# ngrabaskas/Torch-Automatic-Distributed-Neural-Network

Measured on AMD Instinct MI355X. Metric: samples/sec whole-node ResNet-50 DP + GPT-2 PP at 1/2/4/8 MI355X; scaling eff, higher is better.
Workload: dtype bf16

## Files before the change

madnn/ops/__init__.py:

```python
from __future__ import annotations

import os
import threading
from pathlib import Path
from typing import Optional, Sequence

import torch
import torch.nn.functional as F

from . import reference

HERE = Path(__file__).resolve().parent
_KERNELS = HERE / "_madnn_kernels.so"
_lock = threading.Lock()
_loaded = {"kernels": False, "error": None}


def kernels_path() -> Path:
    return _KERNELS


class StaleKernelsError(RuntimeError):
    """The in-tree kernel library was built from different sources than the tree holds."""

# ... 545 lines not shown
    return torch.cat([a * c - b * sn, b * c + a * sn], -1).to(x.dtype)


class _RopeQKVFn(torch.autograd.Function):

    @staticmethod
    def forward(ctx, qkv, cos, sin, rot_heads):
        ctx.save_for_backward(cos, sin)
        ctx.rot = rot_heads
        if _is_dev(qkv):
            return torch.ops.madnn.rope_qkv(qkv, cos, sin, rot_heads, False)
        out = qkv.clone()
        out[:, :, :rot_heads] = _rope_rotate(qkv[:, :, :rot_heads], cos, sin, False)
        return out

    @staticmethod
    def backward(ctx, g):
        cos, sin = ctx.saved_tensors
        g = g.contiguous()
        if _is_dev(g):
            torch.ops.madnn.rope_qkv_(g, cos, sin, ctx.rot, True)
        else:
            g = g.clone()
            g[:, :, : ctx.rot] = _rope_rotate(g[:, :, : ctx.rot], cos, sin, True)
        return g, None, None, None


def rope_qkv(qkv: torch.Tensor, cos: torch.Tensor, sin: torch.Tensor, rot_heads: int) -> torch.Tensor:
    if _is_dev(qkv):
        _need_native("rope_qkv")
        if not (qkv.dtype == torch.bfloat16 and qkv.is_contiguous() and qkv.size(-1) % 16 == 0
                and cos.dtype == torch.float32 and cos.is_contiguous()):
            raise ValueError("rope_qkv: needs a contiguous bf16 qkv (D % 16 == 0) and fp32 tables")
        if qkv.data_ptr() % 16:
            qkv = qkv.clone()
        if cos.data_ptr() % 16 or sin.data_ptr() % 16:
            cos, sin = cos.clone(), sin.clone()
    return _RopeQKVFn.apply(qkv, cos, sin, rot_heads)


class _SwiGLUFn(torch.autograd.Function):

    @staticmethod
    def forward(ctx, gu):
        ctx.save_for_backward(gu)
        return torch.ops.madnn.swiglu_fwd(gu)

    @staticmethod
    def backward(ctx, dh):
        (gu,) = ctx.saved_tensors
        if dh.data_ptr() % 16 or not dh.is_contiguous():
            dh = dh.contiguous().clone()
        return torch.ops.madnn.swiglu_bwd(dh, gu)


def swiglu(gu: torch.Tensor) -> torch.Tensor:
    if (_is_dev(gu) and gu.dtype == torch.bfloat16 and gu.is_contiguous() and gu.size(-1) % 16 == 0
            and gu.data_ptr() % 16 == 0):
        _need_native("swiglu")
        return _SwiGLUFn.apply(gu)
    g, u = gu.chunk(2, dim=-1)
    return F.silu(g) * u


def _nhwc(t: torch.Tensor) -> torch.Tensor:
    return t.contiguous(memory_format=torch.channels_last) if t.dim() == 4 else t.contiguous()


def _rows(t: torch.Tensor) -> torch.Tensor:
    return t.permute(0, 2, 3, 1).reshape(-1, t.size(1)) if t.dim() == 4 else t


def conv1x1_route(cin: int, cout: int) -> tuple:
    fwd = "k9" if (cin <= 256 or cout >= 2 * cin) else "miopen"
    if _K9_DGRAD == "narrow":
        dgrad = "k9" if (cin <= 256 and cout <= 512) else "gemm"
    else:
        dgrad = "gemm" if (cout >= 1024 and cout >= 4 * cin) else "k9"
    return fwd, dgrad, _K9_WGRAD


_K9_WGRAD = os.environ.get("MADNN_K9_WGRAD", "miopen")
_K9_DGRAD = os.environ.get("MADNN_K9_DGRAD", "narrow")


def _routed_conv1x1_fwd(fwd: str, x: torch.Tensor, w: torch.Tensor, stats: bool):
    if fwd == "k9":
        return torch.ops.madnn.conv1x1_fwd(x, w, bool(stats))
    y = F.conv2d(x, w) if x.dim() == 4 else torch.mm(x, w.reshape(w.size(0), -1).t())
    return y, x.new_empty((0, 2, w.size(0)), dtype=torch.float32)


def _routed_conv1x1_wgrad(wgrad: str, dy: torch.Tensor, x: torch.Tensor, w: torch.Tensor) -> torch.Tensor:
    return _k9_wgrad(dy, x, w) if wgrad == "k9" else _conv1x1_wgrad_lib(dy, x, w)


def _with_stats(out: torch.Tensor, part: torch.Tensor, stats: bool):
    return (out, part if part.numel() else None) if stats else out


def _like(g: torch.Tensor, y: torch.Tensor) -> torch.Tensor:
    return g if g.dtype == y.dtype and g.stride() == y.stride() else torch.empty_like(y).copy_(g)


class _Conv1x1Fn(torch.autograd.Function):

    @staticmethod
    def forward(ctx, x, w, stats, fork):
        fwd, dgrad, wgrad = conv1x1_route(x.size(1), w.size(0))
        y, part = _routed_conv1x1_fwd(fwd, x, w, stats)
        ctx.save_for_backward(x, w)
        ctx.route = (dgrad, wgrad)
        ctx.fork = fork
        ctx.mark_non_differentiable(part)
        if fork == 2:
            return y, part, x[:, :, ::2, ::2].contiguous(memory_format=torch.channels_last)
        if fork:
            return y, part, x.view_as(x)
        return y, part

    @staticmethod
    def backward(ctx, dy, _dpart, dfork=None):
        x, w = ctx.saved_tensors
        dgrad, wgrad = ctx.route
        dy = _nhwc(dy.to(x.dtype))
        sub = None
        if ctx.fork == 2:
            sub, dfork = dfork, None
        resmask = _attached(dfork, "_madnn_resmask", strict=True)
        res = _nhwc(dfork.to(x.dtype)) if dfork is not None else None
        if resmask is not None and not (ctx.needs_input_grad[0] and dgrad == "k9"):
            res, resmask = _apply_bit_mask(res, resmask), None
        dx = dw = None
        if ctx.needs_input_grad[0]:
            if dgrad == "k9":
                dx = torch.ops.madnn.conv1x1_dgrad(dy, w, res, resmask)
            else:
                w2 = w.reshape(w.size(0), -1)
                if res is not None:
                    dx = res if res._base is None else _nhwc(res.clone())
                    _rows(dx).addmm_(_rows(dy), w2)
                else:
                    dx = torch.empty_like(x)
                    torch.mm(_rows(dy), w2, out=_rows(dx))
        elif res is not None:
            dx = res
        if sub is not None:
            if dx is None:
                dx = torch.zeros_like(x)
            dx[:, :, ::2, ::2].add_(sub.to(dx.dtype))
        if ctx.needs_input_grad[1]:
            dw = _routed_conv1x1_wgrad(wgrad, dy, x, w)
        return dx, dw, None, None


def conv1x1_supported(x: torch.Tensor, w: torch.Tensor) -> bool:
    if x.device.type != "cuda" or x.dtype != torch.bfloat16 or w.dtype != torch.bfloat16 or x.numel() == 0:
        return False
    if x.dim() == 4:
        if not x.is_contiguous(memory_format=torch.channels_last):
            return False
    elif x.dim() != 2 or not x.is_contiguous():
        return False
    cin, cout = x.size(1), w.size(0)
    if w.numel() != cin * cout or w.stride(0) != cin or w.stride(1) != 1:
        return False
    return cin % 64 == 0 and cout % 64 == 0


def conv1x1(x: torch.Tensor, w: torch.Tensor, *, stats: bool = False, fork: bool = False):
    _need_native("conv1x1")
    y, part, *side = _Conv1x1Fn.apply(x, w, stats, fork)
    ret = (y, part if part.numel() else None, *side) if stats else (y, *side)
    return ret[0] if len(ret) == 1 else ret


class _BNReluConv1x1EpiFn(torch.autograd.Function):

    @staticmethod
    def forward(ctx, y, w, bn_w, bn_b, bn, stats_in, want_stats):
        a, mean, invstd, scale, shift, _ = _bn_fwd_train(y, None, bn_w, bn_b, bn, True, stats_in)
        fwd, _, wgrad = conv1x1_route(a.size(1), w.size(0))
        out, part = _routed_conv1x1_fwd(fwd, a, w, want_stats)
        ctx.save_for_backward(y, a, w, bn_w, mean, invstd, scale, shift)
        ctx.wgrad = wgrad
        ctx.mark_non_differentiable(part)
        return out, part

    @staticmethod
    def backward(ctx, dout, _dpart):
        y, a, w, bn_w, mean, invstd, scale, shift = ctx.saved_tensors
        dout = _nhwc(dout.to(y.dtype))
        da, part = torch.ops.madnn.conv1x1_dgrad_bnb(dout, w, y, scale, shift)
        dw = _routed_conv1x1_wgrad(ctx.wgrad, dout, a, w)
        dy, dbw, dbb = torch.ops.madnn.bn_bwd_ext(da, y, bn_w, mean, invstd, scale, shift, part, True)
        need_bn = ctx.needs_input_grad[2] or ctx.needs_input_grad[3]
        return dy, dw, dbw if need_bn else None, dbb if need_bn else None, None, None, None


def bn_relu_conv1x1(y: torch.Tensor, bn, w: torch.Tensor, *, stats_in: Optional[torch.Tensor] = None,
                    stats: bool = False, checked: bool = False):
    if checked or bn_relu_conv1x1_epi_supported(y, bn, w):
        _need_native("bn_relu_conv1x1")
        return _with_stats(*_BNReluConv1x1EpiFn.apply(y, w, bn.weight, bn.bias, bn, stats_in, stats), stats)
    a = bn(y, relu=True, stats=stats_in) if _is_fused_bn(bn) else torch.relu(bn(y))
    if conv1x1_supported(a, w):
        return conv1x1(a, w, stats=stats)
    out = torch.nn.functional.conv2d(a, w.view(w.size(0), -1, 1, 1)) if a.dim() == 4 else torch.mm(
        a, w.reshape(w.size(0), -1).t())
    return (out, None) if stats else out


def bn_relu_conv1x1_epi_supported(y: torch.Tensor, bn, w: torch.Tensor) -> bool:
    return (_BN_DGRAD_EPI and isinstance(y, torch.Tensor) and _bn_trainable(bn)
            and conv1x1_supported(y, w) and bn_supported(y, bn.weight)
            and conv1x1_route(y.size(1), w.size(0))[1] == "k9")


def _k9f_head(y2, w3, bn2_w, bn2_b, bn2, stats_in):
    a2, mean2, invstd2, scale2, shift2, _ = _bn_fwd_train(y2, None, bn2_w, bn2_b, bn2, True, stats_in)
    y3, part = torch.ops.madnn.conv1x1_fwd(a2, w3, True)
    return a2, y3, part, (mean2, invstd2, scale2, shift2)


def _k9f_tail(ctx, da2, part, y2, bn2_w, bn2_stats, dw3, w3, dbw3, dbb3):
    dy2, dbw2, dbb2 = torch.ops.madnn.bn_bwd_ext(da2, y2, bn2_w, *bn2_stats, part, True)
    need2, need3 = (ctx.needs_input_grad[i] or ctx.needs_input_grad[i + 1] for i in (2, 4))
    return (dy2, dw3.to(w3.dtype).view(w3.shape), dbw2 if need2 else None, dbb2 if need2 else None,
            dbw3 if need3 else None, dbb3 if need3 else None)


class _BN2Conv3BN3Fn(torch.autograd.Function):

    @staticmethod
    def forward(ctx, y2, w3, bn2_w, bn2_b, bn3_w, bn3_b, idt, bn2, bn3, stats_in):
        a2, y3, part, bn2_stats = _k9f_head(y2, w3, bn2_w, bn2_b, bn2, stats_in)
        out, mean3, invstd3, scale3, shift3, mask = _bn_fwd_train(y3, idt, bn3_w, bn3_b, bn3, True, part)
        ctx.save_for_backward(y2, a2, w3, y3, mask, bn2_w, *bn2_stats, bn3_w, mean3, invstd3, scale3, shift3)
        return out

    @staticmethod
    def backward(ctx, dout):
        y2, a2, w3, y3, mask, bn2_w, *bn2_stats, bn3_w, mean3, invstd3, scale3, shift3 = ctx.saved_tensors
        dout = _like(dout, y3)
        coef, dbw3, dbb3 = torch.ops.madnn.bn_bwd_coef(dout, y3, mask, bn3_w, mean3, invstd3, scale3, shift3)
        da2, part, dw3 = torch.ops.madnn.bn3_conv3_bwd(dout, y3, mask, coef, w3, a2, y2, *bn2_stats[2:],
                                                       w3.dtype == torch.bfloat16)
        grads = _k9f_tail(ctx, da2, part, y2, bn2_w, bn2_stats, dw3, w3, dbw3, dbb3)
        dres = dout.view_as(dout)
        _attach(dres, "_madnn_resmask", mask)
        return (*grads, dres, None, None, None)


_BN3_CONV3_FUSED = os.environ.get("MADNN_BN3_CONV3_FUSED", "1") != "0"


def _k9f_supported(y2: torch.Tensor, bn2, w3: torch.Tensor, bn3, other: torch.Tensor) -> bool:
    return (_BN3_CONV3_FUSED and isinstance(y2, torch.Tensor) and isinstance(other, torch.Tensor)
            and bn_relu_conv1x1_epi_supported(y2, bn2, w3) and native_available()
            and bool(torch.ops.madnn.bn3_conv3_bwd_supported(y2.size(1), w3.size(0)))
            and conv1x1_route(y2.size(1), w3.size(0))[0] == "k9" and _bn_trainable(bn3)
            and bn3.weight.numel() == w3.size(0) and y2.requires_grad and torch.is_grad_enabled()
            and other.dtype == y2.dtype and other.dim() == y2.dim() and other.size(0) == y2.size(0)
            and other.shape[2:] == y2.shape[2:])


def bn2_conv3_bn3_supported(y2: torch.Tensor, bn2, w3: torch.Tensor, bn3, idt: torch.Tensor) -> bool:
    return (DEFER_RES_MASK and _k9f_supported(y2, bn2, w3, bn3, idt) and _res_mask_deferred(idt)
            and idt.size(1) == w3.size(0) and bn_supported(idt, bn3.weight))


def bn2_conv3_bn3_add_relu(y2: torch.Tensor, bn2, w3: torch.Tensor, bn3, idt: torch.Tensor,
                           stats_in: Optional[torch.Tensor] = None) -> torch.Tensor:
    _need_native("bn2_conv3_bn3_add_relu")
    return _BN2Conv3BN3Fn.apply(y2, w3, bn2.weight, bn2.bias, bn3.weight, bn3.bias, idt, bn2, bn3, stats_in)


class _BN2Conv3BN3DualFn(torch.autograd.Function):

    @staticmethod
    def forward(ctx, y2, w3, bn2_w, bn2_b, bn3_w, bn3_b, xf, w_ds, bnd_w, bnd_b, bn2, bn3, bn_ds, stats_in):
        a2, y3, part, bn2_stats = _k9f_head(y2, w3, bn2_w, bn2_b, bn2, stats_in)
        yd, part_d = torch.ops.madnn.conv1x1_fwd(xf, w_ds, True)
        out, mask, mean3, invstd3, _, _, mean_d, invstd_d, _, _ = torch.ops.madnn.bn_fwd_dual(
            y3, yd, bn3_w, bn3_b, bn3.running_mean, bn3.running_var, bn3.num_batches_tracked, float(bn3.momentum),
            float(bn3.eps), part, bnd_w, bnd_b, bn_ds.running_mean, bn_ds.running_var, bn_ds.num_batches_tracked,
            float(bn_ds.momentum), float(bn_ds.eps), part_d)
        ctx.save_for_backward(y2, a2, w3, y3, xf, w_ds, yd, mask, bn2_w, *bn2_stats, bn3_w, mean3, invstd3, bnd_w,
                              mean_d, invstd_d)
        return out

    @staticmethod
    def backward(ctx, dout):
        (y2, a2, w3, y3, xf, w_ds, yd, mask, bn2_w, *bn2_stats, bn3_w, mean3, invstd3, bnd_w, mean_d,
         invstd_d) = ctx.saved_tensors
        dout = _like(dout, y3)
        coef, dbw3, dbb3, dbwd, dbbd = torch.ops.madnn.bn_bwd_dual_coef(dout, y3, yd, mask, bn3_w, mean3, invstd3,
                                                                        bnd_w, mean_d, invstd_d)
        da2, part, dw3 = torch.ops.madnn.bn3_conv3_bwd(dout, y3, mask, coef[:3], w3, a2, y2, *bn2_stats[2:],
                                                       w3.dtype == torch.bfloat16)
        dxf, _, dwd = torch.ops.madnn.bn3_conv3_bwd(dout, yd, mask, coef[3:], w_ds, xf, None, None, None,
                                                    w_ds.dtype == torch.bfloat16)
        grads = _k9f_tail(ctx, da2, part, y2, bn2_w, bn2_stats, dw3, w3, dbw3, dbb3)
        needd = ctx.needs_input_grad[8] or ctx.needs_input_grad[9]
        return (*grads, dxf, dwd.to(w_ds.dtype).view(w_ds.shape), dbwd if needd else None,
                dbbd if needd else None, None, None, None, None)


_BN3_CONV3_DUAL = os.environ.get("MADNN_BN3_CONV3_DUAL", "1") != "0"


def bn2_conv3_bn3_add_bn_relu_supported(y2: torch.Tensor, bn2, w3: torch.Tensor, bn3, xf: torch.Tensor,
                                        w_ds: torch.Tensor, bn_ds) -> bool:
    return (_BN3_CONV3_DUAL and _k9f_supported(y2, bn2, w3, bn3, xf) and conv1x1_supported(xf, w_ds)
            and xf.size(1) == y2.size(1) and w_ds.size(0) == w3.size(0) and _bn_trainable(bn_ds)
            and bn_ds.weight.numel() == w3.size(0))


def bn2_conv3_bn3_add_bn_relu(y2: torch.Tensor, bn2, w3: torch.Tensor, bn3, xf: torch.Tensor, w_ds: torch.Tensor,
                              bn_ds, stats_in: Optional[torch.Tensor] = None) -> torch.Tensor:
    _need_native("bn2_conv3_bn3_add_bn_relu")
    return _BN2Conv3BN3DualFn.apply(y2, w3, bn2.weight, bn2.bias, bn3.weight, bn3.bias, xf, w_ds, bn_ds.weight,
                                    bn_ds.bias, bn2, bn3, bn_ds, stats_in)


class _BNReluMaxPoolFn(torch.autograd.Function):

    @staticmethod
    def forward(ctx, y, bn_w, bn_b, bn, stats_in, p):
        mean, invstd, scale, shift = torch.ops.madnn.bn_coef(y, bn_w, bn_b, bn.running_mean, bn.running_var,
                                                             bn.num_batches_tracked, float(bn.momentum),
                                                             float(bn.eps), stats_in)
        out, arg = torch.ops.madnn.pool_bn_fwd(y, scale, shift, int(p))
        ctx.save_for_backward(y, arg, bn_w, mean, invstd, scale, shift)
        ctx.p = int(p)
        return out

    @staticmethod
    def backward(ctx, dp):
        y, arg, bn_w, mean, invstd, scale, shift = ctx.saved_tensors
        dy, dw, db = torch.ops.madnn.pool_bn_bwd(dp, arg, y, bn_w, mean, invstd, scale, shift, ctx.p)
        return dy, dw, db, None, None, None


def _bn_relu_maxpool_modules_ok(bn, pool) -> bool:
    return (_POOL_BN and _bn_trainable(bn)
            and _pair(pool.kernel_size) == (3, 3) and _pair(pool.stride) == (2, 2)
            and _pair(pool.padding) in ((1, 1), (0, 0)) and _pair(pool.dilation) == (1, 1)
            and not pool.ceil_mode and not pool.return_indices)


def bn_relu_maxpool_supported(y: torch.Tensor, bn, pool) -> bool:
    return (isinstance(y, torch.Tensor) and y.device.type == "cuda" and y.dtype == torch.bfloat16 and y.dim() == 4
            and y.is_contiguous(memory_format=torch.channels_last) and _bn_relu_maxpool_modules_ok(bn, pool)
            and y.size(1) % 8 == 0 and 256 % (y.size(1) // 8) == 0 and y.numel() < 2 ** 31)


def bn_relu_maxpool(y: torch.Tensor, bn, pool, stats_in: Optional[torch.Tensor] = None):
    if bn_relu_maxpool_supported(y, bn, pool):
        _need_native("bn_relu_maxpool")
        p = pool.padding if isinstance(pool.padding, int) else pool.padding[0]
        return _BNReluMaxPoolFn.apply(y, bn.weight, bn.bias, bn, stats_in, p)
    a = bn(y, relu=True, stats=stats_in) if _is_fused_bn(bn) else torch.relu(bn(y))
    return pool(a)


# ... 668 lines not shown


def linear_tee(x: torch.Tensor, weight: torch.Tensor, bias: Optional[torch.Tensor] = None):
    if not torch.is_grad_enabled() or not _is_dev(x) or weight.shape[0] % 8:
        return F.linear(x, weight, bias if bias is None or bias.dtype == x.dtype else bias.to(x.dtype)), x
    return _LinearTeeFn.apply(x, weight, bias)


class _GeluMLPFn(torch.autograd.Function):

    @staticmethod
    def forward(ctx, x, w1, b1, w2, b2, residual, kind=1):
        a, pre = _gelu_linear_fwd(x, w1, b1, kind)
        ctx.kind = kind
        y = _linear_residual_fwd(a, w2, b2, residual)
        ctx.save_for_backward(x, w1, pre, a, w2)
        ctx.b1_dtype = b1.dtype if b1 is not None else None
        ctx.b2_dtype = b2.dtype if b2 is not None else None
        ctx.bias_dtype = ctx.b2_dtype
        ctx.params = (w1, w2)
        ctx.has_res = residual is not None
        ctx.res_is_x = residual is x
        return y

    @staticmethod
    def backward(ctx, g):
        x, w1, pre, a, w2 = ctx.saved_tensors
        p1, p2 = ctx.params
        ctx.params = None
        need = ctx.needs_input_grad
        db2 = _out_bias_grad(g, ctx.b2_dtype) if ctx.b2_dtype is not None and need[4] else None
        g2 = g.reshape(-1, g.shape[-1])
        if not g2.is_contiguous():
            g2 = g2.contiguous()
        a2 = a.reshape(-1, a.shape[-1])
        dw2 = _weight_grad(g2, a2, p2) if need[3] else None
        dh, db1 = dgrad_dgelu(g2, w2, pre.reshape(-1, pre.shape[-1]), ctx.b1_dtype or g2.dtype, ctx.kind)
        if ctx.b1_dtype is None or not need[2]:
            db1 = None
        x2 = x.reshape(-1, x.shape[-1])
        dw1 = _weight_grad(dh, x2, p1) if need[1] else None
        if ctx.res_is_x and need[0]:
            dx = _dgrad_plus(dh, w1, g2).view(*x.shape[:-1], w1.shape[1])
            return dx, dw1, db1, dw2, db2, None, None
        dx = (dh @ w1).view(*x.shape[:-1], w1.shape[1]) if need[0] else None
        return dx, dw1, db1, dw2, db2, (g if ctx.has_res else None), None


def gelu_mlp(x: torch.Tensor, w1: torch.Tensor, b1: Optional[torch.Tensor], w2: torch.Tensor,
             b2: Optional[torch.Tensor], residual: Optional[torch.Tensor] = None,
             approximate: str = "tanh") -> torch.Tensor:
    if residual is not None and residual.shape[:-1] != x.shape[:-1]:
        raise ValueError("gelu_mlp: residual must have the output's shape")
    if approximate not in GELU_KIND:
        raise ValueError(f"gelu_mlp: approximate must be 'tanh' or 'none', not {approximate!r}")
    if not _is_dev(x) or not torch.is_grad_enabled() or w1.shape[0] % 8 or w2.shape[0] % 8:
        h = F.gelu(F.linear(x, w1, b1), approximate=approximate)
        y = F.linear(h, w2, b2)
        return y + residual if residual is not None else y
    return _GeluMLPFn.apply(x, w1, b1, w2, b2, residual, GELU_KIND[approximate])


def linear(x: torch.Tensor, weight: torch.Tensor, bias: Optional[torch.Tensor] = None, gelu: bool = False,
           force_fn: bool = False, residual: Optional[torch.Tensor] = None):
    if residual is not None and residual.shape[:-1] != x.shape[:-1]:
        raise ValueError("linear: residual must have the output's shape")
    if not torch.is_grad_enabled() or (not force_fn and (not _is_dev(x) or weight.shape[0] % 8)):
        if not torch.is_grad_enabled() and _is_dev(x) and (gelu or residual is not None) and weight.shape[0] % 8 == 0:
            out = _lt_epilogue(x, weight, bias, residual, gelu)
            if out is not None:
                return out[0]
        y = F.linear(x, weight, bias)
        y = F.gelu(y, approximate="tanh") if gelu else y
        return y + residual if residual is not None else y
    return _LinearFn.apply(x, weight, bias, gelu, residual)


__all__ = [
    "bucket_pack", "bucket_unpack", "flat_scale_cast", "sgd_step", "adam_step", "grad_norm", "layer_norm",
    "rms_norm", "batch_norm_act", "bn_supported", "cross_entropy", "attention", "attention_qkvpacked", "attention_supported",
    "max_pool2d", "max_pool_supported", "conv1x1", "conv1x1_route", "batch_norm_add_bn_relu",
    "batch_norm_dual_supported", "bn_relu_conv1x1", "bn_relu_maxpool",
    "bn_relu_maxpool_supported", "bn_relu_conv3x3", "bn_relu_conv3x3_supported",
    "bn_relu_conv1x1_epi_supported", "bn2_conv3_bn3_add_relu", "bn2_conv3_bn3_supported", "bn2_conv3_bn3_add_bn_relu", "bn2_conv3_bn3_add_bn_relu_supported", "conv1x1_supported", "stem_conv", "stem_supported", "stem_bn_relu_maxpool", "stem_bn_relu_maxpool_supported", "native_available", "load_kernels", "kernels_path", "hidden_supported", "reference",
    "linear", "linear_tee", "gelu_mlp", "bias_grad", "gelu_tanh", "grad_sink", "wgrad_into", "tuned_wgrad", "dgrad",
    "dgrad_dgelu", "load_tuning_table", "export_choices", "sync_choices", "tuning_timings", "tuning_measurements",
]

if os.environ.get("MADNN_EAGER_LOAD", "0") == "1":
    load_kernels()

load_tuning_table()
```

madnn/ops/csrc/conv.hip:

```cpp
#include "mfma.h"

namespace madnn {
namespace conv {

using namespace mf;

constexpr int kThreads = 256;
constexpr int kBK = 64;
constexpr int kTargetWG = 2 * kNumCU;

struct Tune {
  int fwd_wg = kTargetWG;
  int wgrad_wg = 2 * kNumCU;
  int xcd = 1;
};
inline Tune& tune() {
  static Tune t;
  return t;
}

enum Mode : int { kStoreT = 0, kSplit = 1 };

struct GemmArgs {
  const uint16_t* a;
  const uint16_t* b;
  void* out;
  const uint16_t* res;
  const unsigned char* resmask;
  float* stats;
  const uint16_t* bny;
  const float* bnsc;
  const float* bnsh;
  int64_t lda, ldb, ldo;
  int64_t I, J, K;
  int i_tiles, j_tiles, j_groups, k_chunk;
  int xcd;
};

template <bool COL, int R>
struct Stage {
  static constexpr int PER = R / 32;
  u32x4 r[PER];

  __device__ __forceinline__ void load(const uint16_t* __restrict__ base, int64_t ld, int64_t x0, int64_t xlim,
                                       int64_t k0, int64_t klim, int tid) {
#pragma unroll
    for (int i = 0; i < PER; ++i) {
      const int c = tid + kThreads * i;
      int64_t row, lim, col;
      if constexpr (COL) {
        row = k0 + c / (R / 8);
        lim = klim;
        col = x0 + (c % (R / 8)) * 8;
      } else {
        row = x0 + (c >> 3);
        lim = xlim;
        col = k0 + (c & 7) * 8;
      }
      const bool ok = row < lim;
      const u32x4 v = *reinterpret_cast<const u32x4*>(base + (ok ? row : lim - 1) * ld + col);
      const unsigned keep = ok ? 0xffffffffu : 0u;
      r[i] = v & keep;
    }
  }

  __device__ __forceinline__ void store(uint16_t* tile, int tid) const {
#pragma unroll
    for (int i = 0; i < PER; ++i) {
      const int c = tid + kThreads * i;
      int boff;
      if constexpr (COL) {
        boff = swz<R>(c / (R / 8), c % (R / 8));
      } else {
        boff = swz<64>(c >> 3, c & 7);
      }
      *reinterpret_cast<u32x4*>(reinterpret_cast<char*>(tile) + boff) = r[i];
    }
  }

  static __device__ __forceinline__ bf16x8 frag(const uint16_t* tile, int s, int x, int lane) {
    if constexpr (COL) {
      return lds_col<R>(tile, 16 * s, x, lane);
    } else {
      return lds_row(tile, x + (lane & 31), 2 * s + (lane >> 5));
    }
  }
};

template <bool A_COL, bool B_COL, int BI, int BJ, int MODE, bool STATS, bool BNB = false>
__global__ __launch_bounds__(kThreads, 2) void gemm_kernel(const GemmArgs p) {
  static_assert(!(STATS && BNB), "one statistics epilogue per launch");
  constexpr int NI = (BI == 64 && BJ == 64) ? 1 : 2;
  constexpr int WI = BI / (32 * NI), WJ = 4 / WI, NJ = BJ / (32 * WJ);
  static_assert(WI * WJ == 4 && NJ >= 1, "four waves tile the workgroup");
  constexpr int AE = BI * kBK, BE = BJ * kBK, SE = AE + BE;
  static_assert(SE >= BI * BJ, "a pipeline buffer holds the bf16 output tile");
  constexpr int CPR = BI / 8;
// ... 127 lines not shown
                v[e] = (unsigned)f32_to_bf16(lo) | ((unsigned)f32_to_bf16(hi) << 16);
              }
            }
            *reinterpret_cast<u32x4*>(out + j * p.ldo + i0 + 8 * c) = v;
            if constexpr (BNB) {
              const u32x4 yv = *reinterpret_cast<const u32x4*>(p.bny + j * p.ldo + i0 + 8 * c);
#pragma unroll
              for (int e = 0; e < 4; ++e) {
#pragma unroll
                for (int hf = 0; hf < 2; ++hf) {
                  const int k = 2 * e + hf;
                  const float g = bf16_to_f32((unsigned short)(hf ? v[e] >> 16 : v[e] & 0xffffu));
                  const float yy = bf16_to_f32((unsigned short)(hf ? yv[e] >> 16 : yv[e] & 0xffffu));
                  const bool on = yy * bs[k] + bh[k] > 0.f;
                  const float gm = on ? g : 0.f;
                  ssum[k] += gm;
                  ssq[k] += gm * yy;
                }
              }
            }
            if constexpr (STATS) {
#pragma unroll
              for (int e = 0; e < 4; ++e) {
                const float x0 = bf16_to_f32((unsigned short)(v[e] & 0xffffu));
                const float x1 = bf16_to_f32((unsigned short)(v[e] >> 16));
                ssum[2 * e] += x0;
                ssq[2 * e] += x0 * x0;
                ssum[2 * e + 1] += x1;
                ssq[2 * e + 1] += x1 * x1;
              }
            }
          }
        }
      } else {
        const int64_t jw = (int64_t)jt * BJ + wj * NJ * 32 + l32;
        float* out = static_cast<float*>(p.out) + (int64_t)(grp / p.j_tiles) * p.I * p.ldo;
#pragma unroll
        for (int a = 0; a < NI; ++a)
#pragma unroll
          for (int b = 0; b < NJ; ++b)
#pragma unroll
            for (int r = 0; r < 16; ++r) {
              const int64_t i = i0 + (wi * NI + a) * 32 + acc_row(r, hh);
              out[i * p.ldo + jw + b * 32] = acc[a][b][r];
            }
      }
#pragma unroll
      for (int a = 0; a < NI; ++a)
#pragma unroll
        for (int b = 0; b < NJ; ++b) acc[a][b] = zero16();
    }
    if (!more) break;
    __syncthreads();
    cur ^= 1;
    jt = njt;
    ks = nks;
  }

  if constexpr (STATS || BNB) {
    __syncthreads();
    float* red = reinterpret_cast<float*>(smem);
    const int c = tid % CPR, rg = tid / CPR;
#pragma unroll
    for (int e = 0; e < 8; ++e) {
      red[(rg * 2) * BI + 8 * c + e] = ssum[e];
      red[(rg * 2 + 1) * BI + 8 * c + e] = ssq[e];
    }
    __syncthreads();
    for (int k = tid; k < 2 * BI; k += kThreads) {
      const int which = k / BI, ii = k % BI;
      float v = 0.f;
      for (int g = 0; g < RPP; ++g) v += red[(g * 2 + which) * BI + ii];
      p.stats[((int64_t)grp * 2 + which) * p.I + i0 + ii] = v;
    }
  }
}

template <bool A_COL, bool B_COL, int BI, int BJ, int MODE, bool STATS, bool BNB = false>
hipError_t launch(const GemmArgs& p, int grid, hipStream_t s) {
  hipLaunchKernelGGL((gemm_kernel<A_COL, B_COL, BI, BJ, MODE, STATS, BNB>), dim3(grid), dim3(kThreads), 0, s, p);
  return hipGetLastError();
}

inline void plan_persistent(GemmArgs& p, int64_t J, int BI, int64_t I, int64_t K) {
  p.i_tiles = (int)(I / BI);
  p.j_tiles = (int)((J + 127) / 128);
  const int64_t total = (int64_t)p.i_tiles * p.j_tiles;
  const int64_t per = K >= 8 * kBK ? 1 : (total + tune().fwd_wg - 1) / tune().fwd_wg;
  p.j_groups = (int)((p.j_tiles + per - 1) / per);
  p.k_chunk = 0;
}

template <bool BF16>
__global__ __launch_bounds__(256) void split_reduce_kernel(const float* __restrict__ slab, int splits, int64_t n,
                                                           void* __restrict__ dw) {
  const int64_t n4 = n / 4;
  for (int64_t v = (int64_t)blockIdx.x * 256 + threadIdx.x; v < n4; v += (int64_t)gridDim.x * 256) {
    f32x4 acc = reinterpret_cast<const f32x4*>(slab)[v];
    for (int s = 1; s < splits; ++s) acc += reinterpret_cast<const f32x4*>(slab + (int64_t)s * n)[v];
    if constexpr (BF16) {
      const unsigned lo = (unsigned)f32_to_bf16(acc[0]) | ((unsigned)f32_to_bf16(acc[1]) << 16);
      const unsigned hi = (unsigned)f32_to_bf16(acc[2]) | ((unsigned)f32_to_bf16(acc[3]) << 16);
      reinterpret_cast<u32x2*>(dw)[v] = u32x2{lo, hi};
    } else {
      reinterpret_cast<f32x4*>(dw)[v] = acc;
    }
  }
}

inline void wgrad_split(int64_t M, int64_t cin, int64_t cout, int& bi, int& bj, int64_t& tiles, int& k_chunk,
                        int64_t& splits) {
  bi = cout % 128 == 0 ? 128 : 64;
  bj = cin % 128 == 0 ? 128 : 64;
  tiles = (cout / bi) * (cin / bj);
  const int64_t nk = (M + kBK - 1) / kBK;
  splits = (tune().wgrad_wg + tiles - 1) / tiles;
  splits = splits < 1 ? 1 : (splits > nk ? nk : splits);
  k_chunk = (int)((nk + splits - 1) / splits);
  splits = (nk + k_chunk - 1) / k_chunk;
}

constexpr int kFC = 64, kFC4 = 256, kFBM = 128;
constexpr int kFW = kFC4 * kFC, kFT = kFBM * 64;

struct FusedArgs {
  const uint16_t* dout;
  const uint16_t* y;
  const unsigned char* mask;
  const float* coef;
  const uint16_t* w;
  const uint16_t* a;
  const uint16_t* y2;
  const float* sc2;
  const float* sh2;
  uint16_t* da;
  float* partial;
  float* slabs;
  int64_t M;
  int m_tiles;
};

template <bool BNB>
__global__ __launch_bounds__(kThreads, 2) void bn3_conv3_bwd_kernel(const FusedArgs p) {
  __shared__ __attribute__((aligned(16))) uint16_t smem[kFW + 3 * kFT];
  uint16_t* const wt = smem;
  uint16_t* const dyt = smem + kFW;
  uint16_t* const at = dyt + 2 * kFT;
  const int tid = threadIdx.x, wave = tid >> 6, lane = tid & 63, l32 = lane & 31, hh = lane >> 5;
  const int G = gridDim.x;
  const int c8 = tid & 7, r8 = tid >> 3;

  {
    Stage<false, kFBM> sw;
#pragma unroll
    for (int h = 0; h < kFC4 / kFBM; ++h) {
      sw.load(p.w, kFC, h * kFBM, kFC4, 0, kFC, tid);
      sw.store(wt + h * kFT, tid);
    }
  }
  float ssum[BNB ? 8 : 1], ssq[BNB ? 8 : 1];
#pragma unroll
  for (int e = 0; e < (BNB ? 8 : 1); ++e) ssum[e] = ssq[e] = 0.f;
  f32x16 accw[kFC4 / 64], accd[2];
#pragma unroll
  for (int q = 0; q < kFC4 / 64; ++q) accw[q] = zero16();
  accd[0] = accd[1] = zero16();
// ... 137 lines not shown
#pragma unroll
          for (int u = 0; u < 4; ++u) {
            const int r = r8 + 32 * u;
            if (r < valid) {
              const unsigned off = opaque(((unsigned)r * kFC + 8 * c8) * 2u);
              const u32x4 v = *reinterpret_cast<const u32x4*>(ot + opaque((unsigned)out_off(r8, c8)) + 4096 * u);
              *reinterpret_cast<u32x4*>(bo + off) = v;
              const u32x4 yv = *reinterpret_cast<const u32x4*>(by2 + off);
#pragma unroll
              for (int e = 0; e < 4; ++e) {
#pragma unroll
                for (int hf = 0; hf < 2; ++hf) {
                  const int k = 2 * e + hf;
                  const float g = bf16_to_f32((unsigned short)(hf ? v[e] >> 16 : v[e] & 0xffffu));
                  const float yy = bf16_to_f32((unsigned short)(hf ? yv[e] >> 16 : yv[e] & 0xffffu));
                  const float gm = yy * bs[k] + bh[k] > 0.f ? g : 0.f;
                  ssum[k] += gm;
                  ssq[k] += gm * yy;
                }
              }
            }
          }
        } else {
          const int64_t m0 = (int64_t)tile * kFBM;
          const int valid = (int)min((int64_t)kFBM, p.M - m0);
          char* bo = reinterpret_cast<char*>(p.da + m0 * kFC);
#pragma unroll
          for (int u = 0; u < 4; ++u) {
            const int r = r8 + 32 * u;
            if (r < valid)
              *reinterpret_cast<u32x4*>(bo + opaque(((unsigned)r * kFC + 8 * c8) * 2u)) =
                  *reinterpret_cast<const u32x4*>(ot + opaque((unsigned)out_off(r8, c8)) + 4096 * u);
          }
        }
      }
      if (!go) break;
      __syncthreads();
      cur ^= 1;
    }
    if (!more) break;
    tile = ntile;
  }

  const int t2 = (int)opaque(threadIdx.x), w2 = t2 >> 6, col2 = t2 & 31, h2 = (t2 >> 5) & 1;
  float* slab = p.slabs + (int64_t)blockIdx.x * kFW;
#pragma unroll
  for (int q = 0; q < kFC4 / 64; ++q)
#pragma unroll
    for (int r = 0; r < 16; ++r)
      slab[(q * 64 + (w2 >> 1) * 32 + acc_row(r, h2)) * kFC + (w2 & 1) * 32 + col2] = accw[q][r];
  if constexpr (BNB) {
    __syncthreads();
    float* red = reinterpret_cast<float*>(dyt);
    const int rg = t2 >> 3, cg = t2 & 7;
#pragma unroll
    for (int e = 0; e < 8; ++e) {
      red[(rg * 2) * kFC + 8 * cg + e] = ssum[e];
      red[(rg * 2 + 1) * kFC + 8 * cg + e] = ssq[e];
    }
    __syncthreads();
    if (t2 < 2 * kFC) {
      const int which = t2 / kFC, ii = t2 % kFC;
      float v = 0.f;
      for (int g = 0; g < 32; ++g) v += red[(g * 2 + which) * kFC + ii];
      p.partial[((int64_t)blockIdx.x * 2 + which) * kFC + ii] = v;
    }
  }
}

inline int fused_groups(int64_t M) {
  const int64_t tiles = (M + kFBM - 1) / kFBM;
  const int64_t want = tune().fwd_wg < 1 ? 1 : tune().fwd_wg;
  return (int)(tiles < want ? tiles : want);
}

}
}

using namespace madnn::conv;

extern "C" {

int madnn_conv1x1_tune(int key, int value) {
  int* f = key == 0 ? &tune().fwd_wg : key == 1 ? &tune().wgrad_wg : key == 2 ? &tune().xcd : nullptr;
  if (f == nullptr) return -1;
  const int old = *f;
  if (value >= 0) *f = value;
  return old;
}

int madnn_conv1x1_supported(int64_t cin, int64_t cout) {
  return (cin % 64 == 0 && cout % 64 == 0 && cin >= 64 && cout >= 64 && cin <= 16384 && cout <= 16384) ? 1 : 0;
}

int madnn_conv1x1_stat_rows(int64_t M, int64_t cin, int64_t cout) {
  if (!madnn_conv1x1_supported(cin, cout) || M <= 0) return 0;
  GemmArgs p{};
  plan_persistent(p, M, cout % 128 == 0 ? 128 : 64, cout, cin);
  return p.j_groups;
}

int madnn_conv1x1_dgrad_rows(int64_t M, int64_t cin, int64_t cout) {
  if (!madnn_conv1x1_supported(cin, cout) || M <= 0) return 0;
  GemmArgs p{};
  plan_persistent(p, M, cin % 128 == 0 ? 128 : 64, cin, cout);
  return p.j_groups;
}

hipError_t madnn_conv1x1_fwd(const void* x, const void* w, void* y, float* stats, int64_t M, int64_t cin,
                             int64_t cout, hipStream_t s) {
  if (!madnn_conv1x1_supported(cin, cout)) return hipErrorInvalidValue;
  if (M <= 0) return hipSuccess;
  GemmArgs p{};
  p.a = static_cast<const uint16_t*>(w);
  p.lda = cin;
  p.b = static_cast<const uint16_t*>(x);
  p.ldb = cin;
  p.out = y;
  p.ldo = cout;
  p.stats = stats;
  p.xcd = tune().xcd;
  p.I = cout;
  p.J = M;
  p.K = cin;
  const bool wide = cout % 128 == 0;
  plan_persistent(p, M, wide ? 128 : 64, cout, cin);
  const int grid = p.i_tiles * p.j_groups;
  if (wide) {
    return stats ? launch<false, false, 128, 128, kStoreT, true>(p, grid, s)
                 : launch<false, false, 128, 128, kStoreT, false>(p, grid, s);
  }
  return stats ? launch<false, false, 64, 128, kStoreT, true>(p, grid, s)
               : launch<false, false, 64, 128, kStoreT, false>(p, grid, s);
}

hipError_t madnn_conv1x1_dgrad(const void* dy, const void* w, void* dx, const void* res, int64_t M, int64_t cin,
                               int64_t cout, const void* bny, const float* bnsc, const float* bnsh, float* partial,
                               hipStream_t s, const unsigned char* resmask) {
  if (!madnn_conv1x1_supported(cin, cout)) return hipErrorInvalidValue;
  if (M <= 0) return hipSuccess;
  GemmArgs p{};
  p.a = static_cast<const uint16_t*>(w);
  p.lda = cin;
  p.b = static_cast<const uint16_t*>(dy);
  p.ldb = cout;
  p.out = dx;
  p.res = static_cast<const uint16_t*>(res);
  p.resmask = res != nullptr ? resmask : nullptr;
  p.xcd = tune().xcd;
  p.ldo = cin;
  p.I = cin;
  p.J = M;
  p.K = cout;
  const bool wide = cin % 128 == 0;
  plan_persistent(p, M, wide ? 128 : 64, cin, cout);
  const int grid = p.i_tiles * p.j_groups;
  if (bny != nullptr) {
    if (partial == nullptr || bnsc == nullptr || bnsh == nullptr || res != nullptr) return hipErrorInvalidValue;
    p.bny = static_cast<const uint16_t*>(bny);
    p.bnsc = bnsc;
    p.bnsh = bnsh;
    p.stats = partial;
    return wide ? launch<true, false, 128, 128, kStoreT, false, true>(p, grid, s)
                : launch<true, false, 64, 128, kStoreT, false, true>(p, grid, s);
  }
  return wide ? launch<true, false, 128, 128, kStoreT, false>(p, grid, s)
              : launch<true, false, 64, 128, kStoreT, false>(p, grid, s);
}

int64_t madnn_conv1x1_wgrad_ws(int64_t M, int64_t cin, int64_t cout) {
  int bi, bj, kc;
  int64_t tiles, splits;
  wgrad_split(M, cin, cout, bi, bj, tiles, kc, splits);
  return splits * cin * cout;
}

hipError_t madnn_conv1x1_wgrad(const void* dy, const void* x, void* dw, int dw_bf16, float* ws, int64_t M, int64_t cin,
                               int64_t cout, hipStream_t s) {
  if (!madnn_conv1x1_supported(cin, cout)) return hipErrorInvalidValue;
  if (M <= 0) return hipMemsetAsync(dw, 0, (size_t)(cin * cout) * (dw_bf16 ? 2 : 4), s);
  GemmArgs p{};
  p.a = static_cast<const uint16_t*>(dy);
  p.lda = cout;
  p.b = static_cast<const uint16_t*>(x);
  p.ldb = cin;
  p.xcd = tune().xcd;
  p.ldo = cin;
  p.I = cout;
  p.J = cin;
  p.K = M;
  int bi, bj;
  int64_t tiles, splits;
  wgrad_split(M, cin, cout, bi, bj, tiles, p.k_chunk, splits);
  if (ws == nullptr) return hipErrorInvalidValue;
  p.out = ws;
  p.i_tiles = (int)(cout / bi);
  p.j_tiles = (int)(cin / bj);
  const int grid = (int)(tiles * splits);
  p.j_groups = 0;
  hipError_t e;
  if (bi == 128 && bj == 128) e = launch<true, true, 128, 128, kSplit, false>(p, grid, s);
  else if (bi == 128) e = launch<true, true, 128, 64, kSplit, false>(p, grid, s);
  else if (bj == 128) e = launch<true, true, 64, 128, kSplit, false>(p, grid, s);
  else e = launch<true, true, 64, 64, kSplit, false>(p, grid, s);
  if (e != hipSuccess) return e;
  const int64_t n = cin * cout;
  const int64_t blocks = (n / 4 + 255) / 256;
  const dim3 grid_r((unsigned)(blocks < 4 * madnn::kNumCU ? blocks : 4 * madnn::kNumCU));
  if (dw_bf16) {
    hipLaunchKernelGGL(split_reduce_kernel<true>, grid_r, dim3(256), 0, s, ws, (int)splits, n, dw);
  } else {
    hipLaunchKernelGGL(split_reduce_kernel<false>, grid_r, dim3(256), 0, s, ws, (int)splits, n, dw);
  }
  return hipGetLastError();
}

int madnn_bn3_conv3_bwd_supported(int64_t c, int64_t c4) { return (c == kFC && c4 == kFC4) ? 1 : 0; }

int madnn_bn3_conv3_bwd_groups(int64_t M) { return M > 0 ? fused_groups(M) : 0; }

hipError_t madnn_bn3_conv3_bwd(const void* dout, const void* y, const unsigned char* mask, const float* coef,
                               const void* w, const void* a, const void* y2, const float* sc2, const float* sh2,
                               void* da, float* partial, float* slabs, void* dw, int dw_bf16, int64_t M, int64_t c,
                               int64_t c4, hipStream_t s) {
  if (!madnn_bn3_conv3_bwd_supported(c, c4) || M <= 0) return hipErrorInvalidValue;
  const bool bnb = y2 != nullptr;
  if (bnb != (sc2 != nullptr) || bnb != (sh2 != nullptr) || bnb != (partial != nullptr)) return hipErrorInvalidValue;
  FusedArgs p{};
  p.dout = static_cast<const uint16_t*>(dout);
  p.y = static_cast<const uint16_t*>(y);
  p.mask = mask;
  p.coef = coef;
  p.w = static_cast<const uint16_t*>(w);
  p.a = static_cast<const uint16_t*>(a);
  p.y2 = static_cast<const uint16_t*>(y2);
  p.sc2 = sc2;
  p.sh2 = sh2;
  p.da = static_cast<uint16_t*>(da);
  p.partial = partial;
  p.slabs = slabs;
  p.M = M;
  p.m_tiles = (int)((M + kFBM - 1) / kFBM);
  const int grid = fused_groups(M);
  if (bnb) {
    hipLaunchKernelGGL(bn3_conv3_bwd_kernel<true>, dim3(grid), dim3(kThreads), 0, s, p);
  } else {
    hipLaunchKernelGGL(bn3_conv3_bwd_kernel<false>, dim3(grid), dim3(kThreads), 0, s, p);
  }
// ... 14 lines not shown
```

Measured before the change: 14250.

## Add ring-buffered persistent conv1x1 kernel keeping weight slice resident in LDS

Adds a new persistent GEMM kernel for small-K 1x1 convolutions. It loads the whole weight slice into LDS once, then streams activation tiles through a three-stage LDS ring using direct global-to-LDS loads. The output epilogue, including residual, stats and BN-backward fusions, overlaps with the next tile's loads through counted vmcnt waits. Forward tile width switches to 64 for mid-sized K so the resident slice fits. This aims to remove repeated weight reloads and load stalls, at the risk of more LDS use, inline-asm fragility and a Python ctypes call on every k9 op.

After: 14480 (median of 6 runs). +1.6%, better.

```diff
diff --git a/madnn/ops/__init__.py b/madnn/ops/__init__.py
--- a/madnn/ops/__init__.py
+++ b/madnn/ops/__init__.py
@@ -651,11 +651,27 @@
 
 _K9_WGRAD = os.environ.get("MADNN_K9_WGRAD", "miopen")
 _K9_DGRAD = os.environ.get("MADNN_K9_DGRAD", "narrow")
+K9_RING = os.environ.get("MADNN_K9_RING", "1") != "0"
+_K9_TUNE = []
+
+
+def conv1x1_tune(key: int, value: int = -1) -> int:
+    _need_native("conv1x1_tune")
+    if not _K9_TUNE:
+        import ctypes
+
+        _K9_TUNE.append(ctypes.CDLL(str(_KERNELS)).madnn_conv1x1_tune)
+    return int(_K9_TUNE[0](int(key), int(value)))
+
+
+def _k9():
+    conv1x1_tune(3, 1 if K9_RING else 0)
+    return torch.ops.madnn
 
 
 def _routed_conv1x1_fwd(fwd: str, x: torch.Tensor, w: torch.Tensor, stats: bool):
     if fwd == "k9":
-        return torch.ops.madnn.conv1x1_fwd(x, w, bool(stats))
+        return _k9().conv1x1_fwd(x, w, bool(stats))
     y = F.conv2d(x, w) if x.dim() == 4 else torch.mm(x, w.reshape(w.size(0), -1).t())
     return y, x.new_empty((0, 2, w.size(0)), dtype=torch.float32)
 
@@ -703,7 +719,7 @@
         dx = dw = None
         if ctx.needs_input_grad[0]:
             if dgrad == "k9":
-                dx = torch.ops.madnn.conv1x1_dgrad(dy, w, res, resmask)
+                dx = _k9().conv1x1_dgrad(dy, w, res, resmask)
             else:
                 w2 = w.reshape(w.size(0), -1)
                 if res is not None:
@@ -760,7 +776,7 @@
     def backward(ctx, dout, _dpart):
         y, a, w, bn_w, mean, invstd, scale, shift = ctx.saved_tensors
         dout = _nhwc(dout.to(y.dtype))
-        da, part = torch.ops.madnn.conv1x1_dgrad_bnb(dout, w, y, scale, shift)
+        da, part = _k9().conv1x1_dgrad_bnb(dout, w, y, scale, shift)
         dw = _routed_conv1x1_wgrad(ctx.wgrad, dout, a, w)
         dy, dbw, dbb = torch.ops.madnn.bn_bwd_ext(da, y, bn_w, mean, invstd, scale, shift, part, True)
         need_bn = ctx.needs_input_grad[2] or ctx.needs_input_grad[3]
@@ -788,7 +804,7 @@
 
 def _k9f_head(y2, w3, bn2_w, bn2_b, bn2, stats_in):
     a2, mean2, invstd2, scale2, shift2, _ = _bn_fwd_train(y2, None, bn2_w, bn2_b, bn2, True, stats_in)
-    y3, part = torch.ops.madnn.conv1x1_fwd(a2, w3, True)
+    y3, part = _k9().conv1x1_fwd(a2, w3, True)
     return a2, y3, part, (mean2, invstd2, scale2, shift2)
 
 
@@ -850,7 +866,7 @@
     @staticmethod
     def forward(ctx, y2, w3, bn2_w, bn2_b, bn3_w, bn3_b, xf, w_ds, bnd_w, bnd_b, bn2, bn3, bn_ds, stats_in):
         a2, y3, part, bn2_stats = _k9f_head(y2, w3, bn2_w, bn2_b, bn2, stats_in)
-        yd, part_d = torch.ops.madnn.conv1x1_fwd(xf, w_ds, True)
+        yd, part_d = _k9().conv1x1_fwd(xf, w_ds, True)
         out, mask, mean3, invstd3, _, _, mean_d, invstd_d, _, _ = torch.ops.madnn.bn_fwd_dual(
             y3, yd, bn3_w, bn3_b, bn3.running_mean, bn3.running_var, bn3.num_batches_tracked, float(bn3.momentum),
             float(bn3.eps), part, bnd_w, bnd_b, bn_ds.running_mean, bn_ds.running_var, bn_ds.num_batches_tracked,
@@ -1685,7 +1701,7 @@
     "max_pool2d", "max_pool_supported", "conv1x1", "conv1x1_route", "batch_norm_add_bn_relu",
     "batch_norm_dual_supported", "bn_relu_conv1x1", "bn_relu_maxpool",
     "bn_relu_maxpool_supported", "bn_relu_conv3x3", "bn_relu_conv3x3_supported",
-    "bn_relu_conv1x1_epi_supported", "bn2_conv3_bn3_add_relu", "bn2_conv3_bn3_supported", "bn2_conv3_bn3_add_bn_relu", "bn2_conv3_bn3_add_bn_relu_supported", "conv1x1_supported", "stem_conv", "stem_supported", "stem_bn_relu_maxpool", "stem_bn_relu_maxpool_supported", "native_available", "load_kernels", "kernels_path", "hidden_supported", "reference",
+    "bn_relu_conv1x1_epi_supported", "bn2_conv3_bn3_add_relu", "bn2_conv3_bn3_supported", "bn2_conv3_bn3_add_bn_relu", "bn2_conv3_bn3_add_bn_relu_supported", "conv1x1_supported", "conv1x1_tune", "stem_conv", "stem_supported", "stem_bn_relu_maxpool", "stem_bn_relu_maxpool_supported", "native_available", "load_kernels", "kernels_path", "hidden_supported", "reference",
     "linear", "linear_tee", "gelu_mlp", "bias_grad", "gelu_tanh", "grad_sink", "wgrad_into", "tuned_wgrad", "dgrad",
     "dgrad_dgelu", "load_tuning_table", "export_choices", "sync_choices", "tuning_timings", "tuning_measurements",
 ]
diff --git a/madnn/ops/csrc/conv.hip b/madnn/ops/csrc/conv.hip
--- a/madnn/ops/csrc/conv.hip
+++ b/madnn/ops/csrc/conv.hip
@@ -1,3 +1,5 @@
+#include <cstdlib>
+
 #include "mfma.h"
 
 namespace madnn {
@@ -13,6 +15,11 @@
   int fwd_wg = kTargetWG;
   int wgrad_wg = 2 * kNumCU;
   int xcd = 1;
+  int ring = ring_default();
+  static int ring_default() {
+    const char* e = getenv("MADNN_K9_RING");
+    return e != nullptr && *e != 0 ? atoi(e) : 1;
+  }
 };
 inline Tune& tune() {
   static Tune t;
@@ -306,6 +313,302 @@
   return hipGetLastError();
 }
 
+constexpr int kRingStages = 3;
+constexpr int kBStage = 128 * kBK;
+
+__device__ __forceinline__ void glds16_off(const void* base, unsigned voff, unsigned lds_byte) {
+  const unsigned lds = __builtin_amdgcn_readfirstlane(lds_byte);
+  unsigned keep;
+  asm volatile(
+      "s_nop 4\n\ts_mov_b32 %0, m0\n\ts_mov_b32 m0, %3\n\ts_nop 0\n\tglobal_load_lds_dwordx4 %1, %2\n\ts_mov_b32 m0, %0"
+      : "=&s"(keep)
+      : "v"(voff), "s"(base), "s"(lds)
+      : "memory");
+}
+
+__device__ __forceinline__ void ring_bar() {
+  asm volatile("s_waitcnt lgkmcnt(0)" ::: "memory");
+  __builtin_amdgcn_sched_barrier(0);
+  __builtin_amdgcn_s_barrier();
+  __builtin_amdgcn_sched_barrier(0);
+}
+
+template <int N>
+__device__ __forceinline__ void vmcnt() {
+  asm volatile("s_waitcnt vmcnt(%0)" ::"n"(N) : "memory");
+}
+
+template <int EST>
+__device__ __forceinline__ void wait_vm(bool next, int epilogues) {
+  if (next) {
+    if (epilogues == 0) vmcnt<4>();
+    else if (epilogues == 1) vmcnt<4 + EST>();
+    else vmcnt<4 + 2 * EST>();
+  } else {
+    if (epilogues == 0) vmcnt<0>();
+    else if (epilogues == 1) vmcnt<EST>();
+    else vmcnt<2 * EST>();
+  }
+}
+
+template <bool A_COL, int BI, bool STATS, bool BNB>
+__global__ __launch_bounds__(kThreads, 2) void ring_kernel(const GemmArgs p) {
+  static_assert(!(STATS && BNB), "one statistics epilogue per launch");
+  static_assert(!A_COL || BI == 128, "the column image of the weight slice is 128 wide");
+  constexpr int BJ = 128, NS = kRingStages, AK = 256 / BI;
+  constexpr int NI = 2, WI = BI / 64, WJ = 4 / WI, NJ = BJ / (32 * WJ);
+  constexpr int AE = BI * kBK;
+  constexpr int CPR = BI / 8;
+  constexpr int RPP = kThreads / CPR;
+  constexpr int EST = BJ / RPP;
+  constexpr int PR = kBStage / BI;
+  constexpr int NP = BJ / PR;
+  static_assert(NP == 1 || NP == WJ, "a staging pass is the j rows of one wave row");
+  __shared__ __attribute__((aligned(16))) uint16_t smem[AK * AE + NS * kBStage];
+  uint16_t* const ares = smem;
+  uint16_t* const bring = smem + AK * AE;
+  const unsigned lds_a = (unsigned)(size_t)(lds_void*)smem, lds_b = lds_a + 2u * AK * AE;
+  const int tid = threadIdx.x, lane = tid & 63, l32 = lane & 31, hh = lane >> 5;
+  const int wave = __builtin_amdgcn_readfirstlane(tid >> 6);
+  const int wi = wave / WJ, wj = wave % WJ;
+  int wid = blockIdx.x;
+  if (p.xcd) {
+    const int n = gridDim.x, x = wid % 8, q8 = n / 8, r8 = n % 8;
+    wid = (x < r8 ? x * (q8 + 1) : r8 * (q8 + 1) + (x - r8) * q8) + wid / 8;
+  }
+  const int it = wid % p.i_tiles;
+  const int grp = wid / p.i_tiles;
+  const int64_t i0 = (int64_t)it * BI;
+  const int nk = (int)(p.K / kBK);
+  const int jstride = p.j_groups, jtiles = p.j_tiles;
+  int jt = grp;
+  if (jt >= jtiles) return;
+  const int total = ((jtiles - grp + jstride - 1) / jstride) * nk;
+  const uint16_t* const pb = p.b;
+  const int64_t J = p.J, ldb = p.ldb;
+
+  for (int t = 0; t < nk; ++t) {
+#pragma unroll
+    for (int q = 0; q < BI / 32; ++q) {
+      const int inst = wave * (BI / 32) + q;
+      unsigned off;
+      if constexpr (A_COL) {
+        const int r = inst * 4 + (lane >> 4);
+        const int ch = (lane & 15) ^ (((r & 3) << 2) | ((r >> 2) & 3));
+        off = (unsigned)((t * kBK + r) * (int)p.lda + (int)i0 + 8 * ch) * 2u;
+      } else {
+        const int r = inst * 8 + (lane >> 3);
+        const int ch = (lane & 7) ^ ((((r >> 1) & 1) << 2) | ((r >> 2) & 3));
+        off = (unsigned)(((int)i0 + r) * (int)p.lda + t * kBK + 8 * ch) * 2u;
+      }
+      glds16_off(p.a, off, lds_a + 2u * (unsigned)(t * AE + inst * 512));
+    }
+  }
+
+  const int rq0 = wave * 32 + (lane >> 3);
+  unsigned colb[4];
+#pragma unroll
+  for (int q = 0; q < 4; ++q) {
+    const int r = rq0 + 8 * q;
+    colb[q] = 16u * (unsigned)((lane & 7) ^ ((((r >> 1) & 1) << 2) | ((r >> 2) & 3)));
+  }
+  int ijt = grp, ikt = 0, istage = 0;
+  auto issue_b = [&]() {
+    const int64_t j0 = (int64_t)ijt * BJ;
+    const int valid = (int)min((int64_t)BJ, J - j0);
+    const uint16_t* base = pb + j0 * ldb + (int64_t)ikt * kBK;
+    const unsigned dst = lds_b + 2u * (unsigned)(istage * kBStage + wave * 2048);
+#pragma unroll
+    for (int q = 0; q < 4; ++q) {
+      const int row = min(rq0 + 8 * q, valid - 1);
+      glds16_off(base, (unsigned)(row * (int)ldb) * 2u + colb[q], dst + 1024u * q);
+    }
+    istage = istage + 1 == NS ? 0 : istage + 1;
+    if (++ikt == nk) {
+      ikt = 0;
+      ijt += jstride;
+    }
+  };
+  issue_b();
+  if (total > 1) issue_b();
+
+  f32x16 acc[NI][NJ];
+#pragma unroll
+  for (int a = 0; a < NI; ++a)
+#pragma unroll
+    for (int b = 0; b < NJ; ++b) acc[a][b] = zero16();
+  float ssum[8], ssq[8], bs[8], bh[8];
+  if constexpr (STATS || BNB) {
+#pragma unroll
+    for (int e = 0; e < 8; ++e) ssum[e] = ssq[e] = 0.f;
+  }
+  if constexpr (BNB) {
+    const int cc = tid % (BI / 8);
+#pragma unroll
+    for (int e = 0; e < 8; ++e) {
+      bs[e] = p.bnsc[i0 + 8 * cc + e];
+      bh[e] = p.bnsh[i0 + 8 * cc + e];
+    }
+  }
+  auto out_off = [](int r, int c) {
+    if constexpr (BI == 128) return r * 256 + 16 * (c ^ (r & 15));
+    else return r * 128 + 16 * (c ^ ((r >> 1) & 7));
+  };
+
+  int u = 0, t = 0, st = 0;
+  int l1 = 0, l2 = 0;
+  for (;;) {
+    wait_vm<EST>(u + 1 < total, l1 + l2);
+    ring_bar();
+    if (u + 2 < total) issue_b();
+    const uint16_t* abuf = ares + t * AE;
+    uint16_t* bbuf = bring + st * kBStage;
+#pragma unroll
+    for (int s = 0; s < kBK / 16; ++s) {
+      bf16x8 af[NI], bv[NJ];
+#pragma unroll
+      for (int a = 0; a < NI; ++a) af[a] = Stage<A_COL, BI>::frag(abuf, s, (wi * NI + a) * 32, lane);
+#pragma unroll
+      for (int b = 0; b < NJ; ++b) bv[b] = Stage<false, BJ>::frag(bbuf, s, (wj * NJ + b) * 32, lane);
+#pragma unroll
+      for (int a = 0; a < NI; ++a)
+#pragma unroll
+        for (int b = 0; b < NJ; ++b) acc[a][b] = mfma(af[a], bv[b], acc[a][b]);
+    }
+    const bool last = t == nk - 1;
+    if (last) {
+      ring_bar();
+      char* ot = reinterpret_cast<char*>(bbuf);
+      uint16_t* out = static_cast<uint16_t*>(p.out);
+      const int c = tid % CPR;
+#pragma unroll
+      for (int h = 0; h < NP; ++h) {
+        if (NP == 1 || wj == h) {
+#pragma unroll
+          for (int b = 0; b < NJ; ++b) {
+            const int jr = (wj * NJ + b) * 32 + l32 - h * PR;
+#pragma unroll
+            for (int a = 0; a < NI; ++a)
+#pragma unroll
+              for (int g = 0; g < 4; ++g) {
+                const int ic = (wi * NI + a) * 32 + 8 * g + 4 * hh;
+                const unsigned lo = (unsigned)f32_to_bf16(acc[a][b][4 * g]) |
+                                    ((unsigned)f32_to_bf16(acc[a][b][4 * g + 1]) << 16);
+                const unsigned hi = (unsigned)f32_to_bf16(acc[a][b][4 * g + 2]) |
+                                    ((unsigned)f32_to_bf16(acc[a][b][4 * g + 3]) << 16);
+                *reinterpret_cast<u32x2*>(ot + out_off(jr, ic >> 3) + 8 * ((ic >> 2) & 1)) = u32x2{lo, hi};
+              }
+          }
+        }
+        ring_bar();
+#pragma unroll
+        for (int uu = 0; uu < EST / NP; ++uu) {
+          const int r = tid / CPR + RPP * (h * (EST / NP) + uu);
+          const int64_t j = (int64_t)jt * BJ + r;
+          if (j < p.J) {
+            u32x4 v = *reinterpret_cast<const u32x4*>(ot + out_off(r - h * PR, c));
+            if (p.res != nullptr) {
+              u32x4 rv = *reinterpret_cast<const u32x4*>(p.res + j * p.ldo + i0 + 8 * c);
+              if (p.resmask != nullptr) {
+                const unsigned bits = p.resmask[(j * p.ldo + i0 + 8 * c) >> 3];
+#pragma unroll
+                for (int e = 0; e < 4; ++e)
+                  rv[e] &= ((bits >> (2 * e)) & 1u ? 0xffffu : 0u) | ((bits >> (2 * e + 1)) & 1u ? 0xffff0000u : 0u);
+              }
+#pragma unroll
+              for (int e = 0; e < 4; ++e) {
+                const float lo = bf16_to_f32((unsigned short)(v[e] & 0xffffu)) +
+                                 bf16_to_f32((unsigned short)(rv[e] & 0xffffu));
+                const float hi = bf16_to_f32((unsigned short)(v[e] >> 16)) + bf16_to_f32((unsigned short)(rv[e] >> 16));
+                v[e] = (unsigned)f32_to_bf16(lo) | ((unsigned)f32_to_bf16(hi) << 16);
+              }
+            }
+            *reinterpret_cast<u32x4*>(out + j * p.ldo + i0 + 8 * c) = v;
+            if constexpr (BNB) {
+              const u32x4 yv = *reinterpret_cast<const u32x4*>(p.bny + j * p.ldo + i0 + 8 * c);
+#pragma unroll
+              for (int e = 0; e < 4; ++e) {
+#pragma unroll
+                for (int hf = 0; hf < 2; ++hf) {
+                  const int k = 2 * e + hf;
+                  const float g = bf16_to_f32((unsigned short)(hf ? v[e] >> 16 : v[e] & 0xffffu));
+                  const float yy = bf16_to_f32((unsigned short)(hf ? yv[e] >> 16 : yv[e] & 0xffffu));
+                  const bool on = yy * bs[k] + bh[k] > 0.f;
+                  const float gm = on ? g : 0.f;
+                  ssum[k] += gm;
+                  ssq[k] += gm * yy;
+                }
+              }
+            }
+            if constexpr (STATS) {
+#pragma unroll
+              for (int e = 0; e < 4; ++e) {
+                const float x0 = bf16_to_f32((unsigned short)(v[e] & 0xffffu));
+                const float x1 = bf16_to_f32((unsigned short)(v[e] >> 16));
+                ssum[2 * e] += x0;
+                ssq[2 * e] += x0 * x0;
+                ssum[2 * e + 1] += x1;
+                ssq[2 * e + 1] += x1 * x1;
+              }
+            }
+          }
+        }
+        if (h + 1 < NP) ring_bar();
+      }
+#pragma unroll
+      for (int a = 0; a < NI; ++a)
+#pragma unroll
+        for (int b = 0; b < NJ; ++b) acc[a][b] = zero16();
+    }
+    if (++u == total) break;
+    l2 = l1;
+    l1 = last ? 1 : 0;
+    st = st + 1 == NS ? 0 : st + 1;
+    if (last) {
+      t = 0;
+      jt += jstride;
+    } else {
+      ++t;
+    }
+  }
+
+  if constexpr (STATS || BNB) {
+    ring_bar();
+    float* red = reinterpret_cast<float*>(bring);
+    const int c = tid % CPR, rg = tid / CPR;
+#pragma unroll
+    for (int e = 0; e < 8; ++e) {
+      red[(rg * 2) * BI + 8 * c + e] = ssum[e];
+      red[(rg * 2 + 1) * BI + 8 * c + e] = ssq[e];
+    }
+    ring_bar();
+    for (int k = tid; k < 2 * BI; k += kThreads) {
+      const int which = k / BI, ii = k % BI;
+      float v = 0.f;
+      for (int g = 0; g < RPP; ++g) v += red[(g * 2 + which) * BI + ii];
+      p.stats[((int64_t)grp * 2 + which) * p.I + i0 + ii] = v;
+    }
+  }
+}
+
+template <bool A_COL, int BI, bool STATS, bool BNB = false>
+hipError_t launch_ring(const GemmArgs& p, int grid, hipStream_t s) {
+  hipLaunchKernelGGL((ring_kernel<A_COL, BI, STATS, BNB>), dim3(grid), dim3(kThreads), 0, s, p);
+  return hipGetLastError();
+}
+
+inline bool use_ring(bool a_col, int bi, int64_t K) {
+  if (tune().ring <= 0 || (a_col && bi != 128)) return false;
+  const int64_t nk = K / kBK;
+  return bi == 128 ? nk <= 2 : (nk >= 2 && nk <= 4);
+}
+
+inline int fwd_bi(int64_t cin, int64_t cout) {
+  if (cout % 128 != 0) return 64;
+  const int64_t nk = cin / kBK;
+  return (tune().ring > 0 && nk >= 3 && nk <= 4) ? 64 : 128;
+}
+
 inline void plan_persistent(GemmArgs& p, int64_t J, int BI, int64_t I, int64_t K) {
   p.i_tiles = (int)(I / BI);
   p.j_tiles = (int)((J + 127) / 128);
@@ -609,7 +912,11 @@
 extern "C" {
 
 int madnn_conv1x1_tune(int key, int value) {
-  int* f = key == 0 ? &tune().fwd_wg : key == 1 ? &tune().wgrad_wg : key == 2 ? &tune().xcd : nullptr;
+  int* f = key == 0   ? &tune().fwd_wg
+           : key == 1 ? &tune().wgrad_wg
+           : key == 2 ? &tune().xcd
+           : key == 3 ? &tune().ring
+                      : nullptr;
   if (f == nullptr) return -1;
   const int old = *f;
   if (value >= 0) *f = value;
@@ -623,7 +930,7 @@
 int madnn_conv1x1_stat_rows(int64_t M, int64_t cin, int64_t cout) {
   if (!madnn_conv1x1_supported(cin, cout) || M <= 0) return 0;
   GemmArgs p{};
-  plan_persistent(p, M, cout % 128 == 0 ? 128 : 64, cout, cin);
+  plan_persistent(p, M, fwd_bi(cin, cout), cout, cin);
   return p.j_groups;
 }
 
@@ -650,13 +957,16 @@
   p.I = cout;
   p.J = M;
   p.K = cin;
-  const bool wide = cout % 128 == 0;
+  const bool wide = fwd_bi(cin, cout) == 128;
   plan_persistent(p, M, wide ? 128 : 64, cout, cin);
   const int grid = p.i_tiles * p.j_groups;
+  const bool ring = use_ring(false, wide ? 128 : 64, cin);
   if (wide) {
+    if (ring) return stats ? launch_ring<false, 128, true>(p, grid, s) : launch_ring<false, 128, false>(p, grid, s);
     return stats ? launch<false, false, 128, 128, kStoreT, true>(p, grid, s)
                  : launch<false, false, 128, 128, kStoreT, false>(p, grid, s);
   }
+  if (ring) return stats ? launch_ring<false, 64, true>(p, grid, s) : launch_ring<false, 64, false>(p, grid, s);
   return stats ? launch<false, false, 64, 128, kStoreT, true>(p, grid, s)
                : launch<false, false, 64, 128, kStoreT, false>(p, grid, s);
 }
@@ -682,15 +992,18 @@
   const bool wide = cin % 128 == 0;
   plan_persistent(p, M, wide ? 128 : 64, cin, cout);
   const int grid = p.i_tiles * p.j_groups;
+  const bool ring = use_ring(true, wide ? 128 : 64, cout);
   if (bny != nullptr) {
     if (partial == nullptr || bnsc == nullptr || bnsh == nullptr || res != nullptr) return hipErrorInvalidValue;
     p.bny = static_cast<const uint16_t*>(bny);
     p.bnsc = bnsc;
     p.bnsh = bnsh;
     p.stats = partial;
+    if (ring) return launch_ring<true, 128, false, true>(p, grid, s);
     return wide ? launch<true, false, 128, 128, kStoreT, false, true>(p, grid, s)
                 : launch<true, false, 64, 128, kStoreT, false, true>(p, grid, s);
   }
+  if (ring) return launch_ring<true, 128, false>(p, grid, s);
   return wide ? launch<true, false, 128, 128, kStoreT, false>(p, grid, s)
               : launch<true, false, 64, 128, kStoreT, false>(p, grid, s);
 }
```
